# IceLab-X/FidelityFusion

Measured on AMD Instinct MI355X. Metric: GP NLML+Cholesky throughput (NxN fp64 GF/s, %MFMA-roofline) at N=16384, higher is better.
Workload: dtype f64; 1 GPU; headline: single-fidelity cigp NLML forward, ARD kernel, 1 block of N=16384 D=16 d=1 (BASELINE configs[2]); N=16384, D=16, d=1, blocks=1, blocks_in_flight_per_rank=1, parallelism=fidelity-shard x1 (LPT partition, one 8-byte all-reduce per step)

## Files before the change

fidelityfusion_amd/csrc/ffgp_internal.h:

```cpp
#pragma once
#include <hip/hip_runtime.h>
#include <cstdint>
#include <cstdio>
#include <cstdlib>
#include <cstring>
#include <vector>

#include "../../include/ffgp.h"

typedef double d4_t __attribute__((ext_vector_type(4)));
typedef double d2_t __attribute__((ext_vector_type(2)));

#define FFGP_NB 128
#define FFGP_MAX_STAGES 16

#define FFGP_HIP(call)                                                                        \
  do {                                                                                        \
    hipError_t e_ = (call);                                                                   \
    if (e_ != hipSuccess) {                                                                   \
      fprintf(stderr, "[ffgp] HIP error %s at %s:%d\n", hipGetErrorString(e_), __FILE__, __LINE__); \
      return FFGP_ERR_HIP;                                                                    \
    }                                                                                         \
  } while (0)

#define FFGP_CHECK(call)            \
  do {                              \
    int s_ = (call);                \
    if (s_ != 0) return s_;         \
  } while (0)

#define FFGP_GRAD_LANES 4
static inline int ffgp_round_up(int x, int m) { return (x + m - 1) / m * m; }

__device__ __forceinline__ double ffgp_kfun_val(int kind, double rinv, double s) {
  if (kind == FFGP_KFUN_SE) return exp(-0.5 * s);
  if (kind == FFGP_KFUN_MATERN12) return exp(-sqrt(s) * rinv);
  if (kind == FFGP_KFUN_MATERN32) {
    const double a = sqrt(3.0 * s) * rinv;
    return (1.0 + a) * exp(-a);
  }
  if (kind == FFGP_KFUN_RQ) return pow(1.0 + 0.5 * s * rinv, -1.0 / rinv);
  const double a = sqrt(5.0 * s) * rinv;
  return (1.0 + a + (5.0 / 3.0) * s * rinv * rinv) * exp(-a);
}
__device__ __forceinline__ double ffgp_kfun_m2d(int kind, double rinv, double s) {
  if (kind == FFGP_KFUN_SE) return exp(-0.5 * s);
  if (kind == FFGP_KFUN_MATERN12) {
    const double r = sqrt(s);
    return rinv / r * exp(-r * rinv);
  }
  if (kind == FFGP_KFUN_MATERN32) return 3.0 * rinv * rinv * exp(-sqrt(3.0 * s) * rinv);
  if (kind == FFGP_KFUN_RQ) return pow(1.0 + 0.5 * s * rinv, -1.0 / rinv - 1.0);
  const double a = sqrt(5.0 * s) * rinv;
  return (5.0 / 3.0) * rinv * rinv * (1.0 + a) * exp(-a);
}
__device__ __forceinline__ double ffgp_kfun_dparam(int kind, double rinv, double s, double phi) {
  if (kind != FFGP_KFUN_RQ) return 0.0;
  const double u = 0.5 * s * rinv;
  return phi * (u / (1.0 + u) - log1p(u));
}

__attribute__((weak)) __constant__ double ffgp_exp_coef[14] = {1.0, 1.0, 0.5, 1.0 / 6, 1.0 / 24, 1.0 / 120, 1.0 / 720, 1.0 / 5040, 1.0 / 40320, 1.0 / 362880,
                                         1.0 / 3628800, 1.0 / 39916800, 1.0 / 479001600, 1.0 / 6227020800.0};
struct ExpCoef {
  double c[14];
};
__device__ __forceinline__ void ffgp_exp_load(ExpCoef& e) {
#pragma unroll
  for (int i = 0; i < 14; ++i) e.c[i] = ffgp_exp_coef[i];
}
__device__ __forceinline__ double ffgp_exp_fast(double x, const ExpCoef& e) {
  x = fmax(x, -750.0);
  const double n = __builtin_rint(x * 1.4426950408889634);
  double r = __builtin_fma(n, -6.93147180369123816490e-01, x);
  r = __builtin_fma(n, -1.90821492927058770002e-10, r);
  double p = e.c[13];
#pragma unroll
  for (int i = 12; i >= 0; --i) p = __builtin_fma(p, r, e.c[i]);
  return __builtin_amdgcn_ldexp(p, (int)n);
}

__device__ __forceinline__ int ffgp_pow2_exp(double m) {
  if (!(m > 0.0)) return 0;
  const int e = ((__double2hiint(m) >> 20) & 0x7ff) - 1023;
  return min(max(e, -1021), 1021);
}

enum { OP_KMAJOR = 0, OP_MNMAJOR = 1 };
enum { TILES_FULL = 0, TILES_LOWER = 1 };

struct GemmArgs {
  const double* A;
  const double* B;
  double* C;
  int m, n, k;
  int lda, ldb, ldc;
  double alpha, beta;
// ... 295 lines not shown
```

fidelityfusion_amd/csrc/gemm.hip:

```cpp
#include <algorithm>

#include "ffgp_internal.h"
#include "diag_block.h"

#define BK 16
#ifndef FFGP_PD_SMALL
#define FFGP_PD_SMALL 4
#endif

#ifdef FFGP_GEMM_TRACE
__device__ unsigned long long* ffgp_trace_buf = nullptr;
extern "C" int ffgp_debug_set_trace(void* p) {
  return hipMemcpyToSymbol(HIP_SYMBOL(ffgp_trace_buf), &p, sizeof(p)) == hipSuccess ? 0 : -1;
}
#define FFGP_TRACE(slot)                                                                            \
  do {                                                                                              \
    if (tid == 0 && ffgp_trace_buf) {                                                               \
      ffgp_trace_buf[(size_t)bid * 8 + (slot)] = __builtin_readcyclecounter();                      \
      if ((slot) == 0) {                                                                            \
        unsigned hwid = 0, xcc = 0;                                                                 \
        asm volatile("s_getreg_b32 %0, hwreg(HW_REG_HW_ID)" : "=s"(hwid));                          \
        asm volatile("s_getreg_b32 %0, hwreg(HW_REG_XCC_ID)" : "=s"(xcc));                          \
        ffgp_trace_buf[(size_t)bid * 8 + 6] = ((unsigned long long)xcc << 32) | hwid;               \
        ffgp_trace_buf[(size_t)bid * 8 + 7] = wall_clock64();                                       \
// ... 185 lines not shown
  d4_t acc[WM][WN];
  if (load_c) {
#pragma unroll
    for (int i = 0; i < WM; ++i)
#pragma unroll
      for (int r = 0; r < 4; ++r) {
        const char* rowb = baseC + (size_t)(i * 4 + r) * row4_bytes;
#pragma unroll
        for (int j = 0; j < WN; ++j) acc[i][j][r] = *reinterpret_cast<const double*>(rowb + voffC + j * 128);
      }
  } else {
#pragma unroll
    for (int i = 0; i < WM; ++i)
#pragma unroll
      for (int j = 0; j < WN; ++j) acc[i][j] = (d4_t){0.0, 0.0, 0.0, 0.0};
  }
  sstore<OPA, TM>(smem, tid, ra[0]);
  sstore<OPB, TN>(smem + BUFA, tid, rb[0]);
  __syncthreads();
#ifdef FFGP_GEMM_TRACE
  if (tid == 0 && ffgp_trace_buf) ffgp_trace_buf[(size_t)trace_bid * 8 + 1] = __builtin_readcyclecounter();
#endif
  baseA += (size_t)PD * stepA;
  baseB += (size_t)PD * stepB;
  for (int kt0 = 0; kt0 < nkt; kt0 += PD) {
#pragma unroll
    for (int u = 0; u < PD; ++u) {
      const int kt = kt0 + u;
      if (kt >= nkt) break;
      const int par = (PD == 1) ? (kt & 1) : (u & 1);
      const double* sA = smem + par * STAGE;
      const double* sB = sA + BUFA;
      if (kt + PD < nkt) {
        gload_fast<TM>(baseA, voffA, ra[u]);
        gload_fast<TN>(baseB, voffB, rb[u]);
        baseA += stepA;
        baseB += stepB;
      }
#pragma unroll
      for (int kq = 0; kq < 4; ++kq) {
        double a[WM], b[WN];
#pragma unroll
        for (int i = 0; i < WM; ++i) a[i] = sA[offA[kq] + i * subA];
#pragma unroll
        for (int j = 0; j < WN; ++j) b[j] = sB[offB[kq] + j * subB];
#pragma unroll
        for (int i = 0; i < WM; ++i)
#pragma unroll
          for (int j = 0; j < WN; ++j)
            acc[i][j] = __builtin_amdgcn_mfma_f64_16x16x4f64(a[i], b[j], acc[i][j], 0, 0, NEG ? 1 : 0);
      }
      if (kt + 1 < nkt) {
        double* dA = smem + (par ^ 1) * STAGE;
        sstore<OPA, TM>(dA, tid, ra[(u + 1) % PD]);
        sstore<OPB, TN>(dA + BUFA, tid, rb[(u + 1) % PD]);
      }
      __syncthreads();
    }
  }
#ifdef FFGP_GEMM_TRACE
  if (tid == 0 && ffgp_trace_buf) ffgp_trace_buf[(size_t)trace_bid * 8 + 2] = __builtin_readcyclecounter();
#endif
#pragma unroll
  for (int i = 0; i < WM; ++i)
#pragma unroll
    for (int r = 0; r < 4; ++r) {
      char* rowb = baseC + (size_t)(i * 4 + r) * row4_bytes;
#pragma unroll
      for (int j = 0; j < WN; ++j) *reinterpret_cast<double*>(rowb + voffC + j * 128) = acc[i][j][r];
    }
}

typedef unsigned gemm_v4u __attribute__((ext_vector_type(4)));
__device__ __forceinline__ __amdgpu_buffer_rsrc_t gemm_rsrc(const char* base) {
  return __builtin_amdgcn_make_buffer_rsrc(const_cast<char*>(base), 0, 0xffffffff, 0x00020000);
}
template <int TS>
__device__ __forceinline__ void gload_buf(__amdgpu_buffer_rsrc_t r, const unsigned (&voff)[Geo<TS>::NLD], d2_t (&v)[Geo<TS>::NLD]) {
#pragma unroll
  for (int i = 0; i < Geo<TS>::NLD; ++i) v[i] = __builtin_bit_cast(d2_t, (gemm_v4u)__builtin_amdgcn_raw_buffer_load_b128(r, (int)voff[i], 0, 0));
}

typedef __attribute__((address_space(3))) char gemm_lds_t;
__device__ __forceinline__ void dma_lane_offsets(int tid, const unsigned (&voff)[4], unsigned (&dv)[4]) {
#pragma unroll
  for (int i = 0; i < 4; ++i) {
    const int idx = tid + 256 * i;
    const int row = idx >> 3, slot = idx & 7;
    dv[i] = voff[i] + (unsigned)(((slot ^ ((row >> 1) & 7)) - slot) * 16);
  }
}
__device__ __forceinline__ void gemm_dma16(__amdgpu_buffer_rsrc_t r, gemm_lds_t* dst, unsigned voff, int soff) {
  __builtin_amdgcn_raw_ptr_buffer_load_lds(r, dst, 16, (int)voff, soff, 0, 0);
}
#define DMA_BARRIER() asm volatile("s_waitcnt vmcnt(0) lgkmcnt(0)\n\ts_barrier" ::: "memory")

template <int OPA, int OPB, bool NEG, bool DIAG = false>
__device__ __forceinline__ void gemm_tile_fast128(const char* __restrict__ baseA, const char* __restrict__ baseB, size_t stepA, size_t stepB,
                                                  char* __restrict__ baseC, size_t row4_bytes, unsigned voffC, bool load_c, double* smem,
                                                  int nkt, int tid, const unsigned (&voffA)[4], const unsigned (&voffB)[4],
                                                  const int (&offA)[4], const int (&offB)[4], int trace_bid, double alpha = 0.0,
                                                  double beta = 0.0) {
  constexpr int TS = 128, W = 4;
  const int wave_d = DIAG ? __builtin_amdgcn_readfirstlane(tid >> 6) : 0;
  const bool mma = !DIAG || wave_d != 1;
  constexpr int BUFA = opbuf<OPA, TS>(), BUFB = opbuf<OPB, TS>(), STAGE = BUFA + BUFB;
  constexpr int subA = (OPA == OP_KMAJOR) ? 256 : 16;
  constexpr int subB = (OPB == OP_KMAJOR) ? 256 : 16;
#define GEMM_PIN() __builtin_amdgcn_sched_barrier(0)
#define GEMM_READ(st, kq, a, b)                                         \
  do {                                                                  \
    _Pragma("unroll") for (int i = 0; i < W; ++i) a[i] = (st)[offA[kq] + i * subA];        \
    _Pragma("unroll") for (int j = 0; j < W; ++j) b[j] = (st)[BUFA + offB[kq] + j * subB]; \
    GEMM_PIN();                                                         \
  } while (0)
#define GEMM_MFMA(a, b)                                                 \
  do {                                                                  \
    if (!DIAG || mma) {                                                 \
      _Pragma("unroll") for (int i = 0; i < W; ++i)                     \
        _Pragma("unroll") for (int j = 0; j < W; ++j)                   \
          acc[i][j] = __builtin_amdgcn_mfma_f64_16x16x4f64(a[i], b[j], acc[i][j], 0, 0, NEG ? 1 : 0);  \
    }                                                                   \
    GEMM_PIN();                                                         \
  } while (0)
  constexpr bool DMA = (OPA == OP_KMAJOR && OPB == OP_KMAJOR);
  [[maybe_unused]] const __amdgpu_buffer_rsrc_t rsA = gemm_rsrc(baseA), rsB = gemm_rsrc(baseB);
  [[maybe_unused]] unsigned dvA[4], dvB[4];
  [[maybe_unused]] gemm_lds_t* ldsw = nullptr;
  if constexpr (DMA) {
    dma_lane_offsets(tid, voffA, dvA);
    dma_lane_offsets(tid, voffB, dvB);
    ldsw = (gemm_lds_t*)smem + __builtin_amdgcn_readfirstlane(tid >> 6) * 1024;
  }
#define GEMM_DMA(p, stage, kt)                                          \
  gemm_dma16((p) < 4 ? rsA : rsB, ldsw + (stage) * (STAGE * 8) + ((p) < 4 ? 0 : BUFA * 8) + ((p) & 3) * 4096, \
             (p) < 4 ? dvA[(p) & 3] : dvB[(p) & 3], (kt) * (BK * 8))
#define GEMM_DMA_ALL(stage, kt)                                         \
  do {                                                                  \
    _Pragma("unroll") for (int p_ = 0; p_ < 8; ++p_) GEMM_DMA(p_, stage, kt); \
    GEMM_PIN();                                                         \
  } while (0)
#define GEMM_MFMA_DMA(a, b, stage, kt)                                  \
  do {                                                                  \
    if constexpr (DIAG) {       \
      GEMM_DMA_ALL(stage, kt);                                          \
      GEMM_MFMA(a, b);                                                  \
    } else {                                                            \
      _Pragma("unroll") for (int i = 0; i < W; ++i)                     \
        _Pragma("unroll") for (int j = 0; j < W; ++j) {                 \
          acc[i][j] = __builtin_amdgcn_mfma_f64_16x16x4f64(a[i], b[j], acc[i][j], 0, 0, NEG ? 1 : 0); \
          if (i * W + j < 8) {                                          \
            GEMM_PIN();                                                 \
            GEMM_DMA(i * W + j, stage, kt);                             \
            GEMM_PIN();                                                 \
          }                                                             \
        }                                                               \
      GEMM_PIN();                                                       \
    }                                                                   \
  } while (0)
  [[maybe_unused]] d2_t ra[4], rb[4];
  if constexpr (DMA) {
    GEMM_DMA_ALL(0, 0);
    if (nkt > 1) GEMM_DMA_ALL(1, 1);
  } else {
    gload_buf<TS>(rsA, voffA, ra);
    gload_buf<TS>(rsB, voffB, rb);
  }
  d4_t acc[W][W];
  if (load_c) {
// ... 66 lines not shown
      GEMM_PIN();
      GEMM_READ(sS, 1, ya, yb);
      GEMM_MFMA(xa, xb);
      GEMM_READ(sS, 2, xa, xb);
      GEMM_MFMA(ya, yb);
      sstore<OPA, TS>(sN, tid, ra);
      sstore<OPB, TS>(sN + BUFA, tid, rb);
      GEMM_PIN();
      GEMM_READ(sS, 3, ya, yb);
      GEMM_MFMA(xa, xb);
      LDS_BARRIER();
      GEMM_PIN();
      GEMM_READ(sN, 0, xa, xb);
      GEMM_MFMA(ya, yb);
    }
  }
  {
    const double* sS = smem + ((nkt - 1) & 1) * STAGE;
    GEMM_READ(sS, 1, ya, yb);
    GEMM_MFMA(xa, xb);
    GEMM_READ(sS, 2, xa, xb);
    GEMM_MFMA(ya, yb);
    GEMM_READ(sS, 3, ya, yb);
    GEMM_MFMA(xa, xb);
    GEMM_MFMA(ya, yb);
  }
#undef GEMM_PIN
#undef GEMM_READ
#undef GEMM_MFMA
#undef GEMM_DMA
#undef GEMM_DMA_ALL
#undef GEMM_MFMA_DMA
#ifdef FFGP_GEMM_TRACE
  if (tid == 0 && ffgp_trace_buf) ffgp_trace_buf[(size_t)trace_bid * 8 + 2] = __builtin_readcyclecounter();
#endif
  if constexpr (DIAG) {
    if (!mma) return;
    const bool below = wave_d == 2;
    const int lrow = (tid & 63) >> 4, lcol = tid & 15;
    const bool use_c = (beta != 0.0);
    double cv[2][4][W];
    auto load_group = [&](int i, double (&dst)[4][W]) {
#pragma unroll
      for (int r = 0; r < 4; ++r) {
        const char* rowb = baseC + (size_t)(i * 4 + r) * row4_bytes;
#pragma unroll
        for (int j = 0; j < W; ++j) dst[r][j] = *reinterpret_cast<const double*>(rowb + voffC + j * 128);
      }
    };
    if (use_c) {
      load_group(0, cv[0]);
    } else {
#pragma unroll
      for (int b = 0; b < 2; ++b)
#pragma unroll
        for (int r = 0; r < 4; ++r)
#pragma unroll
          for (int j = 0; j < W; ++j) cv[b][r][j] = 0.0;
    }
#pragma unroll
    for (int i = 0; i < W; ++i) {
      if (use_c && i + 1 < W) load_group(i + 1, cv[(i + 1) & 1]);
#pragma unroll
      for (int r = 0; r < 4; ++r) {
        char* rowb = baseC + (size_t)(i * 4 + r) * row4_bytes;
#pragma unroll
        for (int j = 0; j < W; ++j)
          if (below || i > j || (i == j && 4 * r + lrow >= lcol))
            *reinterpret_cast<double*>(rowb + voffC + j * 128) = alpha * acc[i][j][r] + beta * cv[i & 1][r][j];
      }
    }
    return;
  }
#pragma unroll
  for (int i = 0; i < W; ++i)
#pragma unroll
    for (int r = 0; r < 4; ++r) {
      char* rowb = baseC + (size_t)(i * 4 + r) * row4_bytes;
#pragma unroll
      for (int j = 0; j < W; ++j) *reinterpret_cast<double*>(rowb + voffC + j * 128) = acc[i][j][r];
    }
}

template <int OPA, int OPB, int TM, int TN, bool GUARD>
__device__ __forceinline__ void gemm_mainloop(const GemmArgs& p, const double* __restrict__ Ag, const double* __restrict__ Bg,
                                              double* smem, int m0, int n0, int kt0, int kt1, int tid,
                                              const int (&offA)[4], const int (&offB)[4],
                                              d4_t (&acc)[Geo<TM>::WT][Geo<TN>::WT]) {
  constexpr int WM = Geo<TM>::WT, WN = Geo<TN>::WT;
  constexpr int BUFA = opbuf<OPA, TM>(), BUFB = opbuf<OPB, TN>(), STAGE = BUFA + BUFB;
  constexpr int subA = (OPA == OP_KMAJOR) ? 256 : 16;
  constexpr int subB = (OPB == OP_KMAJOR) ? 256 : 16;
  d2_t ra[Geo<TM>::NLD], rb[Geo<TN>::NLD];
  gload<OPA, TM, GUARD>(Ag, p.lda, m0, p.m, kt0 * BK, p.k, tid, p.avec != 0, ra);
  gload<OPB, TN, GUARD>(Bg, p.ldb, n0, p.n, kt0 * BK, p.k, tid, p.bvec != 0, rb);
  sstore<OPA, TM>(smem, tid, ra);
  sstore<OPB, TN>(smem + BUFA, tid, rb);
  __syncthreads();
  for (int kt = kt0; kt < kt1; ++kt) {
    const int par = (kt - kt0) & 1;
    const double* sA = smem + par * STAGE;
    const double* sB = sA + BUFA;
    const bool more = (kt + 1 < kt1);
    if (more) {
      gload<OPA, TM, GUARD>(Ag, p.lda, m0, p.m, (kt + 1) * BK, p.k, tid, p.avec != 0, ra);
      gload<OPB, TN, GUARD>(Bg, p.ldb, n0, p.n, (kt + 1) * BK, p.k, tid, p.bvec != 0, rb);
    }
#pragma unroll
    for (int kq = 0; kq < 4; ++kq) {
      double a[WM], b[WN];
#pragma unroll
      for (int i = 0; i < WM; ++i) a[i] = sA[offA[kq] + i * subA];
#pragma unroll
      for (int j = 0; j < WN; ++j) b[j] = sB[offB[kq] + j * subB];
#pragma unroll
      for (int i = 0; i < WM; ++i)
#pragma unroll
        for (int j = 0; j < WN; ++j) acc[i][j] = __builtin_amdgcn_mfma_f64_16x16x4f64(a[i], b[j], acc[i][j], 0, 0, 0);
    }
    if (more) {
      double* dA = smem + (par ^ 1) * STAGE;
      sstore<OPA, TM>(dA, tid, ra);
      sstore<OPB, TN>(dA + BUFA, tid, rb);
    }
    __syncthreads();
  }
}

template <int OPA, int OPB, int MODE, int TM, int TN>
__device__ __forceinline__ void gemm_one_tile(const GemmArgs& p, const double* __restrict__ Ag, const double* __restrict__ Bg,
                                              double* __restrict__ Cg, double* smem, int ti, int tj, const int tid, const int bid,
                                              const bool general = false) {
  constexpr int WM = Geo<TM>::WT, WN = Geo<TN>::WT;
  const int lane = tid & 63, wave = tid >> 6;
  const int wm = wave >> 1, wn = wave & 1;
  int offA[4], offB[4];
  frag_offsets<OPA, TM>(lane, wm * (TM / 2), offA);
  frag_offsets<OPB, TN>(lane, wn * (TN / 2), offB);
  const bool fast_ab = p.fast && p.avec && p.bvec;
  const int m0 = ti * TM, n0 = tj * TN;

  int kbeg = 0, kend = p.k;
  if (p.lo_i) kbeg = max(kbeg, ti * TM);
  if (p.lo_j) kbeg = max(kbeg, tj * TN);
  if (p.hi_i) kend = min(kend, (ti + 1) * TM);
  if (p.hi_j) kend = min(kend, (tj + 1) * TN);
  const int kt0 = kbeg / BK;
  const int kt1 = (kend + BK - 1) / BK;

  const bool interior = (m0 + TM <= p.m) && (n0 + TN <= p.n) && (kt1 * BK <= p.k) && p.avec && p.bvec;
  if constexpr (TM == 128 && TN == 128 && OPA == OP_KMAJOR && OPB == OP_KMAJOR) {
    if (p.pack && fast_ab && interior && kt0 == 0 && kt1 * BK == p.k && !(MODE == TILES_LOWER && m0 < n0 + TN)) return;
  }
  const bool diag = (MODE == TILES_LOWER && m0 < n0 + TN);
  constexpr bool DIAG_FAST = (TM == 128 && TN == 128 && MODE == TILES_LOWER && OPA == OP_KMAJOR && OPB == OP_KMAJOR);
  if (fast_ab && interior && kt0 < kt1 && !general && (!diag || (DIAG_FAST && p.light))) {
    const size_t k0 = (size_t)kt0 * BK;
    const char* bA = reinterpret_cast<const char*>(Ag) +
                     ((OPA == OP_KMAJOR) ? ((size_t)m0 * p.lda + k0) : (k0 * p.lda + m0)) * 8;
    const char* bB = reinterpret_cast<const char*>(Bg) +
                     ((OPB == OP_KMAJOR) ? ((size_t)n0 * p.ldb + k0) : (k0 * p.ldb + n0)) * 8;
    const size_t stepA = (OPA == OP_KMAJOR) ? (size_t)BK * 8 : (size_t)BK * p.lda * 8;
    const size_t stepB = (OPB == OP_KMAJOR) ? (size_t)BK * 8 : (size_t)BK * p.ldb * 8;
    char* bC = reinterpret_cast<char*>(Cg) + ((size_t)m0 * p.ldc + n0) * 8;
    const size_t row4 = (size_t)p.ldc * 32;
    constexpr int PD = (TM == 128) ? 1 : FFGP_PD_SMALL;
    unsigned voffA[Geo<TM>::NLD], voffB[Geo<TN>::NLD];
    lane_byte_offsets<OPA, TM>(p.lda, tid, voffA);
    lane_byte_offsets<OPB, TN>(p.ldb, tid, voffB);
    const unsigned voffC = (unsigned)((wm * (TM / 2) + (lane >> 4)) * p.ldc + wn * (TN / 2) + (lane & 15)) * 8u;
    if constexpr (TM == 128 && TN == 128) {
      if constexpr (DIAG_FAST) {
        if (diag) {
          gemm_tile_fast128<OPA, OPB, false, true>(bA, bB, stepA, stepB, bC, row4, voffC, false, smem, kt1 - kt0, tid, voffA, voffB, offA, offB, bid,
                                                   p.alpha, p.beta);
          FFGP_TRACE(3);
          return;
        }
      }
      if (p.alpha < 0.0)
        gemm_tile_fast128<OPA, OPB, true>(bA, bB, stepA, stepB, bC, row4, voffC, p.beta != 0.0, smem, kt1 - kt0, tid, voffA, voffB, offA, offB, bid);
      else
        gemm_tile_fast128<OPA, OPB, false>(bA, bB, stepA, stepB, bC, row4, voffC, p.beta != 0.0, smem, kt1 - kt0, tid, voffA, voffB, offA, offB, bid);
    } else if (p.alpha < 0.0)
      gemm_tile_fast<OPA, OPB, TM, TN, true, PD>(bA, bB, stepA, stepB, bC, row4, voffC, p.beta != 0.0, smem, kt1 - kt0, tid, voffA,
                                             voffB, offA, offB, bid);
    else
      gemm_tile_fast<OPA, OPB, TM, TN, false, PD>(bA, bB, stepA, stepB, bC, row4, voffC, p.beta != 0.0, smem, kt1 - kt0, tid, voffA,
                                              voffB, offA, offB, bid);
    FFGP_TRACE(3);
    return;
  }

  d4_t acc[WM][WN];
#pragma unroll
  for (int i = 0; i < WM; ++i)
#pragma unroll
    for (int j = 0; j < WN; ++j) acc[i][j] = (d4_t){0.0, 0.0, 0.0, 0.0};

  if (kt0 < kt1) {
    if (interior)
      gemm_mainloop<OPA, OPB, TM, TN, false>(p, Ag, Bg, smem, m0, n0, kt0, kt1, tid, offA, offB, acc);
    else
      gemm_mainloop<OPA, OPB, TM, TN, true>(p, Ag, Bg, smem, m0, n0, kt0, kt1, tid, offA, offB, acc);
  }

  FFGP_TRACE(2);
  const double alpha = p.alpha, beta = p.beta;
  const bool use_c = (beta != 0.0);
  const int rbase0 = m0 + wm * (TM / 2) + (lane >> 4);
  const int cbase = n0 + wn * (TN / 2) + (lane & 15);
  double cv[2][4][WN];
  auto load_group = [&](int i, double (&dst)[4][WN]) {
#pragma unroll
    for (int r = 0; r < 4; ++r) {
      const int rowc = min(rbase0 + i * 16 + 4 * r, p.m - 1);
#pragma unroll
      for (int j = 0; j < WN; ++j) {
        const int colc = min(cbase + j * 16, p.n - 1);
        dst[r][j] = Cg[(size_t)rowc * p.ldc + colc];
      }
    }
  };
  if (use_c) {
    load_group(0, cv[0]);
  } else {
#pragma unroll
    for (int b = 0; b < 2; ++b)
#pragma unroll
      for (int r = 0; r < 4; ++r)
#pragma unroll
        for (int j = 0; j < WN; ++j) cv[b][r][j] = 0.0;
  }
#pragma unroll
  for (int i = 0; i < WM; ++i) {
    if (use_c && i + 1 < WM) load_group(i + 1, cv[(i + 1) & 1]);
#pragma unroll
    for (int r = 0; r < 4; ++r) {
      const int row = rbase0 + i * 16 + 4 * r;
#pragma unroll
      for (int j = 0; j < WN; ++j) {
        const int col = cbase + j * 16;
        if (row < p.m && col < p.n && (MODE != TILES_LOWER || col <= row)) {
          Cg[(size_t)row * p.ldc + col] = alpha * acc[i][j][r] + beta * cv[i & 1][r][j];
        }
      }
    }
  }
  FFGP_TRACE(3);
}

template <int PD>
__device__ __forceinline__ void gemm_slab16(const GemmArgs& p, const double* __restrict__ Ag, const double* __restrict__ Bg,
                                            double* __restrict__ Cg, double* smem, int m0, int n0, const int tid, const int bid) {
  constexpr int BUFA = 16 * 16, BUFB = opbuf<OP_KMAJOR, 128>(), STAGE = BUFA + BUFB;
  static_assert((PD & 1) == 0, "even prefetch depth: the LDS stage parity is compile-time");
  const int lane = tid & 63;
  const int wave = __builtin_amdgcn_readfirstlane(tid >> 6);
  int offA[4], offB[4];
  frag_offsets<OP_KMAJOR, 128>(lane, 0, offA);
  frag_offsets<OP_KMAJOR, 128>(lane, wave * 32, offB);
  const int nkt = p.k / BK;
  const bool has_a = wave < 2;
  const int arow = (tid >> 3) & 15, ach = tid & 7;
  const char* pA = reinterpret_cast<const char*>(Ag) + ((size_t)min(m0 + arow, p.m - 1) * p.lda + ach * 2) * 8;
  const int sa = arow * 16 + ((ach ^ ((arow >> 1) & 7)) << 1);
// ... 34 lines not shown
#pragma unroll
      for (int kq = 0; kq < 4; ++kq) {
        const double a = sA[offA[kq]];
        const double b0 = sB[offB[kq]], b1 = sB[offB[kq] + 256];
        acc[0] = __builtin_amdgcn_mfma_f64_16x16x4f64(a, b0, acc[0], 0, 0, 0);
        acc[1] = __builtin_amdgcn_mfma_f64_16x16x4f64(a, b1, acc[1], 0, 0, 0);
      }
      if (kt + 1 < nkt) {
        double* dA = smem + ((u & 1) ^ 1) * STAGE;
        if (has_a) *reinterpret_cast<d2_t*>(dA + sa) = ra[(u + 1) % PD];
        sstore<OP_KMAJOR, 128>(dA + BUFA, tid, rb[(u + 1) % PD]);
      }
      __syncthreads();
    }
  }
  FFGP_TRACE(2);
  const double alpha = p.alpha, beta = p.beta;
  const bool use_c = (beta != 0.0);
  const int row0 = m0 + (lane >> 4);
  const int col0 = n0 + wave * 32 + (lane & 15);
  double cv[4][2];
#pragma unroll
  for (int r = 0; r < 4; ++r) {
    const int rowc = min(row0 + 4 * r, p.m - 1);
#pragma unroll
    for (int j = 0; j < 2; ++j) cv[r][j] = use_c ? Cg[(size_t)rowc * p.ldc + col0 + j * 16] : 0.0;
  }
#pragma unroll
  for (int r = 0; r < 4; ++r) {
    const int row = row0 + 4 * r;
    if (row < p.m) {
#pragma unroll
      for (int j = 0; j < 2; ++j) Cg[(size_t)row * p.ldc + col0 + j * 16] = alpha * acc[j][r] + beta * cv[r][j];
    }
  }
  FFGP_TRACE(3);
}

template <int OPA, int OPB, int MODE, int TM, int TN>
__device__ __forceinline__ void gemm_block(const GemmArgs& p, const double* __restrict__ Ag, const double* __restrict__ Bg,
                                           double* __restrict__ Cg, double* smem, const int tid, const int bid) {
  FFGP_TRACE(0);
  if constexpr (TM == 128 && TN == 128 && MODE == TILES_LOWER && OPA == OP_KMAJOR && OPB == OP_KMAJOR) {
    if (bid >= p.slab_at) {
      const int s = bid - p.slab_at;
      const int mw = p.tiles_m * 128;
      const int per = (p.m - mw + 15) >> 4;
      const int tj = __builtin_amdgcn_readfirstlane(s / per);
      const int sl = __builtin_amdgcn_readfirstlane(s - tj * per);
      FFGP_TRACE_TILE(p.tiles_m, tj, 16);
      gemm_slab16<FFGP_PD_SMALL>(p, Ag, Bg, Cg, smem, mw + 16 * sl, tj * 128, tid, bid);
      return;
    }
  }
  if constexpr (TM == 128 && TN == 128) {
    if (bid >= p.split_at) {
      const int q = bid - p.split_at;
      int Ti, Tj;
      decode_tile(p.split_at + (q >> 2), MODE, p.tiles_m, p.tiles_n, Ti, Tj, p.band_log2);
      const int ti = __builtin_amdgcn_readfirstlane(2 * Ti + ((q >> 1) & 1));
      const int tj = __builtin_amdgcn_readfirstlane(2 * Tj + (q & 1));
      if (ti * 64 >= p.m || tj * 64 >= p.n || (MODE == TILES_LOWER && tj > ti)) return;
      FFGP_TRACE_TILE(ti, tj, 64);
      gemm_one_tile<OPA, OPB, MODE, 64, 64>(p, Ag, Bg, Cg, smem, ti, tj, tid, bid, MODE == TILES_LOWER && Ti == Tj);
      return;
    }
  }
  int t = bid;
  if (!(p.lo_i | p.lo_j | p.hi_i | p.hi_j)) {
    const int nwg = p.total_tiles;
    const int q = nwg >> 3, r = nwg & 7, xcd = bid & 7;
    t = (xcd < r ? xcd * (q + 1) : r * (q + 1) + (xcd - r) * q) + (bid >> 3);
  }
  int ti, tj;
  decode_tile(t, MODE, p.tiles_m, p.tiles_n, ti, tj, p.band_log2);
  ti = __builtin_amdgcn_readfirstlane(ti);
  tj = __builtin_amdgcn_readfirstlane(tj);
  FFGP_TRACE_TILE(ti, tj, TM);
  gemm_one_tile<OPA, OPB, MODE, TM, TN>(p, Ag, Bg, Cg, smem, ti, tj, tid, bid);
}

template <int OPA, int OPB, int MODE, int TAG, int TM, int TN>
__global__ __launch_bounds__(256, 2) void ffgp_gemm_f64(GemmArgs p) {
  __shared__ __attribute__((aligned(16))) double smem[2 * (opbuf<OPA, TM>() + opbuf<OPB, TN>())];
  const int tid = threadIdx.x;
  if (p.pub_word && tid == 0 && blockIdx.x == 0 && blockIdx.y == 0 && blockIdx.z == 0)
    __hip_atomic_store(p.pub_word, p.pub_val, __ATOMIC_RELAXED, __HIP_MEMORY_SCOPE_SYSTEM);
  if (p.prio) __builtin_amdgcn_s_setprio(2);
  const double* __restrict__ Ag = p.A + (size_t)blockIdx.y * p.sA + (size_t)blockIdx.z * p.sA2;
  const double* __restrict__ Bg = p.B + (size_t)blockIdx.y * p.sB + (size_t)blockIdx.z * p.sB2;
  double* __restrict__ Cg = p.C + (size_t)blockIdx.y * p.sC + (size_t)blockIdx.z * p.sC2;
  gemm_block<OPA, OPB, MODE, TM, TN>(p, Ag, Bg, Cg, smem, tid, blockIdx.x);
}

template <int OPA, int OPB, int MODE, int TAG, int TM, int TN>
__global__ __launch_bounds__(256, 2) void ffgp_gemm_f64_rag(GemmRag q) {
  __shared__ __attribute__((aligned(16))) double smem[2 * (opbuf<OPA, TM>() + opbuf<OPB, TN>())];
  const int tid = threadIdx.x;
  const GemmRagMember& r = q.mem[blockIdx.y];
  if ((int)blockIdx.x >= r.grid) return;
  if (q.base.prio) __builtin_amdgcn_s_setprio(2);
  GemmArgs p = q.base;
  p.A = r.A; p.B = r.B; p.C = r.C;
  p.m = r.m; p.n = r.n; p.k = r.k;
  p.lda = r.lda; p.ldb = r.ldb; p.ldc = r.ldc;
  p.tiles_m = r.tiles_m; p.tiles_n = r.tiles_n; p.total_tiles = r.total_tiles;
  p.grid = r.grid; p.split_at = r.split_at; p.slab_at = r.slab_at; p.light = r.light;
  p.fast = r.fast; p.avec = r.avec; p.bvec = r.bvec;
  gemm_block<OPA, OPB, MODE, TM, TN>(p, p.A, p.B, p.C, smem, tid, blockIdx.x);
}

#define GEMM_BAND_LOG2 3
#define POLITE_PAD_KB 40
template <int OPA, int OPB, int MODE, int TAG, int TM, int TN>
static int launch_t(ffgp_handle* h, const GemmArgs& a) {
  if (a.pad_lds > 0)
    FFGP_HIP(hipFuncSetAttribute(reinterpret_cast<const void*>(&ffgp_gemm_f64<OPA, OPB, MODE, TAG, TM, TN>),
                                 hipFuncAttributeMaxDynamicSharedMemorySize, 64 * 1024));
  hipLaunchKernelGGL((ffgp_gemm_f64<OPA, OPB, MODE, TAG, TM, TN>), dim3(a.grid, a.batch, a.batch2), dim3(256), a.pad_lds, h->stream, a);
  return FFGP_OK;
}

template <int TS>
static int dispatch(ffgp_handle* h, int opa, int opb, int mode, int syrk_tag, const GemmArgs& a) {
  if (syrk_tag) {
    if (opa == OP_KMAJOR && opb == OP_KMAJOR && mode == TILES_LOWER) return launch_t<OP_KMAJOR, OP_KMAJOR, TILES_LOWER, 1, TS, TS>(h, a);
  } else if (mode == TILES_LOWER) {
    if (opa == OP_KMAJOR && opb == OP_KMAJOR) return launch_t<OP_KMAJOR, OP_KMAJOR, TILES_LOWER, 0, TS, TS>(h, a);
    if (opa == OP_MNMAJOR && opb == OP_MNMAJOR) return launch_t<OP_MNMAJOR, OP_MNMAJOR, TILES_LOWER, 0, TS, TS>(h, a);
  } else {
    if (opa == OP_KMAJOR && opb == OP_KMAJOR) return launch_t<OP_KMAJOR, OP_KMAJOR, TILES_FULL, 0, TS, TS>(h, a);
    if (opa == OP_KMAJOR && opb == OP_MNMAJOR) return launch_t<OP_KMAJOR, OP_MNMAJOR, TILES_FULL, 0, TS, TS>(h, a);
    if (opa == OP_MNMAJOR && opb == OP_MNMAJOR) return launch_t<OP_MNMAJOR, OP_MNMAJOR, TILES_FULL, 0, TS, TS>(h, a);
    if (opa == OP_MNMAJOR && opb == OP_KMAJOR) return launch_t<OP_MNMAJOR, OP_KMAJOR, TILES_FULL, 0, TS, TS>(h, a);
  }
  return FFGP_ERR_ARG;
}

static inline bool aligned16(const void* p) { return (reinterpret_cast<uintptr_t>(p) & 15) == 0; }

static int count_tiles(int mode, int m, int n, int tsm, int tsn, int& tm, int& tn) {
  tm = (m + tsm - 1) / tsm;
  tn = (n + tsn - 1) / tsn;
  if (mode != TILES_LOWER) return tm * tn;
  int total = 0;
  for (int ti = 0; ti < tm; ++ti) total += (ti + 1 < tn) ? ti + 1 : tn;
  return total;
}

__global__ __launch_bounds__(256) void ffgp_splitk_reduce(const double* __restrict__ P, int ldp, long sP, int parts, double* __restrict__ C,
                                                         int ldc, int m, int n, double beta) {
  const long e = (long)blockIdx.x * 256 + threadIdx.x;
  if (e >= (long)m * n) return;
  const int r = (int)(e / n), c = (int)(e - (long)r * n);
  double acc = 0.0;
  const double* p = P + (size_t)r * ldp + c;
  for (int s = 0; s < parts; ++s) acc += p[(size_t)s * sP];
  double* dst = C + (size_t)r * ldc + c;
  *dst = (beta != 0.0) ? acc + beta * *dst : acc;
}

static int ensure_skw(ffgp_handle* h, size_t bytes) {
  if (bytes <= h->skw_bytes) return FFGP_OK;
  if (h->skw) {
    hipStreamSynchronize(h->stream);
    if (h->aux) hipStreamSynchronize(h->aux);
    hipFree(h->skw);
  }
  h->skw = nullptr;
  h->skw_bytes = 0;
  const size_t gran = (size_t)16 << 20;
  const size_t want = (bytes + gran - 1) / gran * gran;
  if (hipMalloc(&h->skw, want) != hipSuccess) return FFGP_ERR_ALLOC;
  h->skw_bytes = want;
  ++h->alloc_epoch;
  return FFGP_OK;
}

struct SkinnyArgs {
  const double* A;
// ... 498 lines not shown
```

fidelityfusion_amd/csrc/handle.hip:

```cpp
#include <atomic>
#include <iterator>
#include <cmath>
#include <strings.h>

#include "drivers.h"

#define SCAL_DOUBLES 2048

static const char* k_stage_names[FFGP_MAX_STAGES] = {"assemble", "potrf", "reduce", "trtri", "lauum", "grad",
                                                     "predict_gemm", "", "", "", "", "", "", "", "", ""};

int ffgp_ensure_ws(ffgp_handle* h, size_t bytes) {
  if (bytes <= h->ws_bytes) return FFGP_OK;
  if (h->ws) {
    hipStreamSynchronize(h->stream);
    hipFree(h->ws);
    h->ws = nullptr;
    h->ws_bytes = 0;
  }
  const size_t gran = (size_t)64 << 20;
  const size_t want = (bytes + gran - 1) / gran * gran;
  if (hipMalloc(&h->ws, want) != hipSuccess) {
    fprintf(stderr, "[ffgp] workspace allocation of %zu bytes failed\n", want);
    (void)hipGetLastError();
// ... 95 lines not shown
  for (int i = 0; i <= FFGP_MAX_STAGES; ++i) FFGP_HIP(hipEventCreate(&h->ev[i]));
  FFGP_HIP(hipEventCreate(&h->syrk_ev[0]));
  FFGP_HIP(hipEventCreate(&h->syrk_ev[1]));
  return FFGP_OK;
}

int ffgp_ensure_aux2(ffgp_handle* h) {
  if (h->aux2) return FFGP_OK;
  FFGP_HIP(hipStreamCreateWithFlags(&h->aux2, hipStreamNonBlocking));
  FFGP_HIP(hipStreamCreateWithFlags(&h->aux3, hipStreamNonBlocking));
  for (int i = 0; i < 2; ++i) FFGP_HIP(hipEventCreateWithFlags(&h->tri_ev[i], hipEventDisableTiming));
  return FFGP_OK;
}

extern "C" int ffgp_prepare_streams(ffgp_handle* h) {
  if (!h) return FFGP_ERR_ARG;
  FFGP_HIP(hipSetDevice(h->device));
  FFGP_CHECK(ffgp_ensure_aux2(h));
  FFGP_HIP(hipMemsetAsync(h->d_info + 8, 0, sizeof(int), h->aux));
  FFGP_HIP(hipMemsetAsync(h->d_info + 9, 0, sizeof(int), h->aux2));
  FFGP_HIP(hipMemsetAsync(h->d_info + 10, 0, sizeof(int), h->aux3));
  FFGP_HIP(hipStreamSynchronize(h->aux));
  FFGP_HIP(hipStreamSynchronize(h->aux2));
  FFGP_HIP(hipStreamSynchronize(h->aux3));
  return FFGP_OK;
}

static std::atomic<int> g_live_handles{0};
extern "C++" int ffgp_live_handles() { return g_live_handles.load(std::memory_order_relaxed); }

static bool env_on(const char* key) {
  const char* v = getenv(key);
  return v && *v && strcmp(v, "0") && strcasecmp(v, "false") && strcasecmp(v, "off");
}
static int default_ho_values() {
  const char* f = getenv("FFGP_HANDOFF");
  if (f && !strcmp(f, "events")) return 0;
  if (f && !strcmp(f, "values")) return 1;
  static const char* const serialising[] = {"ROCPROF_COUNTER_COLLECTION", "ROCPROF_COUNTERS", "ROCPROF_COUNTER_GROUPS", "ROCPROF_ADVANCED_THREAD_TRACE",
                                            "ROCP_METRICS", "ROCPROFILER_METRICS_PATH", "HIP_LAUNCH_BLOCKING", "CUDA_LAUNCH_BLOCKING",
                                            "AMD_SERIALIZE_KERNEL", "AMD_SERIALIZE_COPY"};
  for (const char* k : serialising)
    if (env_on(k)) return 0;
  const char* tools = getenv("HSA_TOOLS_LIB");
  if (tools && (strstr(tools, "rocprofiler64") || strstr(tools, "libroctracer"))) return 0;
  return 1;
}

int ffgp_create(int device, ffgp_handle** out) {
  if (!out) return FFGP_ERR_ARG;
  int count = 0;
  if (hipGetDeviceCount(&count) != hipSuccess || count <= 0 || device < 0 || device >= count) {
    fprintf(stderr, "[ffgp] no usable HIP device (requested %d of %d); libffgp has no CPU fallback\n", device, count);
    return FFGP_ERR_NODEVICE;
  }
  FFGP_HIP(hipSetDevice(device));
  ffgp_handle* h = new ffgp_handle();
  h->device = device;
  h->lookahead = 1;
  h->small_tile_threshold = 640;
  h->batch_grad_ob = 1;
  h->tile32_threshold = 1024;
  h->polite_m = 8192;
  h->split_rem_max = 180;
  h->syrk_light_tiles = 1;
  h->super_block = 1024;
  h->splitk_min_k = 1024;
  h->tlin_gemm_min = 8192;
  h->skinny_max_n = 8;
  h->super_min_n = 2048;
  h->la_carry = 2;
  h->la_carry_n = 12288;
  h->la_carry_rows = 8192;
  h->la_min_n = 1024;
  h->chase_xl = 1;
  h->chase_xl_max_n = 2048;
  {
    static std::atomic<int> next_xcc{0};
    h->chase_xcc = next_xcc.fetch_add(1) & 7;
  }
  h->aux_prio = 1;
  h->nb_outer = 512;
  h->trsm128 = 1;
  h->polite64_pad_kb = 60;
  h->polite32_pad_kb = 46;
  h->ho_values = default_ho_values();
  h->ho_defer = 2;
  h->ho_gate = 1;
  h->grad_lanes = 3;
  h->ho_timeout_ms = 2000;
  h->ho_defer_slot = -1;
  h->ho_gdefer_slot = -1;
  h->diag_excl_rows = 4096;
  h->trsm128_max_m = 8192;
  h->trtri_overlap = 1;
  h->small2_off = 1;
  h->q2_split_min_cols = 8192;
  h->sb_lower = 1;
  h->sb_lower_min_n = 6144;
  h->sb_sym_wg = 2048;
  h->asm_mm = 1;
  h->asm_mm_min = 6144;
  h->asm_mm_grid = 768;
  const int rc = create_resources(h);
  if (rc != FFGP_OK) {
    ffgp_destroy(h);
    return rc;
  }
  g_live_handles.fetch_add(1, std::memory_order_relaxed);
  h->counted_live = 1;
  *out = h;
  return FFGP_OK;
}

int ffgp_destroy(ffgp_handle* h) {
  if (!h) return FFGP_OK;
  if (h->counted_live) {
    g_live_handles.fetch_sub(1, std::memory_order_relaxed);
    h->counted_live = 0;
  }
  hipSetDevice(h->device);
  if (h->own) hipStreamSynchronize(h->own);
  if (h->aux) hipStreamSynchronize(h->aux);
  if (h->ws) hipFree(h->ws);
  if (h->dinv) hipFree(h->dinv);
  if (h->sinv) hipFree(h->sinv);
  if (h->tsw) hipFree(h->tsw);
  if (h->skw) hipFree(h->skw);
  if (h->ews) hipFree(h->ews);
  if (h->d_link) hipFree(h->d_link);
  if (h->aux2) hipStreamDestroy(h->aux2);
  if (h->aux3) hipStreamDestroy(h->aux3);
  if (h->ev_switch) hipEventDestroy(h->ev_switch);
  for (int i = 0; i < 2; ++i)
    if (h->tri_ev[i]) hipEventDestroy(h->tri_ev[i]);
  if (h->d_info) hipFree(h->d_info);
  if (h->ho_mem) hipFree(h->ho_mem);
  if (h->bt_info) hipFree(h->bt_info);
  if (h->train_g) hipFree(h->train_g);
  if (h->train_tree) hipFree(h->train_tree);
  for (int z = 0; z < FFGP_GRAD_LANES; ++z) {
    if (h->lane_ev[z]) hipEventDestroy(h->lane_ev[z]);
    if (z > 0 && h->lane_skw[z]) hipFree(h->lane_skw[z]);
  }
  if (h->lane_scal) hipFree(h->lane_scal);
  if (h->small_kbuf) hipFree(h->small_kbuf);
  if (h->train_blk) hipFree(h->train_blk);
  if (h->train_blk_host) hipHostFree(h->train_blk_host);
  ffgp_assemble_collect_free(h);
  if (h->bt_info_host) hipHostFree(h->bt_info_host);
  if (h->d_scal) hipFree(h->d_scal);
  if (h->d_asm) hipFree(h->d_asm);
  ffgp_rawg_drop(h->fwdg);
  if (h->fwdg) {
    if (h->fwdg->stage) hipFree(h->fwdg->stage);
    delete h->fwdg;
    h->fwdg = nullptr;
  }
  if (h->h_info) hipHostFree(h->h_info);
  if (h->h_scal) hipHostFree(h->h_scal);
  for (int i = 0; i <= FFGP_MAX_STAGES; ++i)
    if (h->ev[i]) hipEventDestroy(h->ev[i]);
  for (int i = 0; i < 2; ++i)
    if (h->syrk_ev[i]) hipEventDestroy(h->syrk_ev[i]);
  for (hipEvent_t e : h->syrk_pool) hipEventDestroy(e);
  for (int i = 0; i < 10; ++i)
    if (h->la_ev[i]) hipEventDestroy(h->la_ev[i]);
  if (h->aux) hipStreamDestroy(h->aux);
// ... 139 lines not shown
```

Measured before the change: 55920 GF/s.

## Add multi-stage LDS DMA ring pipeline for 64 and 32 GEMM tiles

Adds a ring-buffered GEMM tile path for 64x64 and 32x32 k-major tiles. It uses buffer-load-to-LDS DMA with a configurable stage count, partial vmcnt waits and explicitly interleaved MFMA and DMA issue. LDS sizing now scales with the stage count, and the polite-kernel LDS padding is derived from it, so total occupancy stays unchanged. With the default ring depth of 2 this mainly replaces the register-staged path with direct DMA. That risks different scheduling behaviour on the small tiles.

```diff
diff --git a/fidelityfusion_amd/csrc/ffgp_internal.h b/fidelityfusion_amd/csrc/ffgp_internal.h
--- a/fidelityfusion_amd/csrc/ffgp_internal.h
+++ b/fidelityfusion_amd/csrc/ffgp_internal.h
@@ -13,6 +13,14 @@
 
 #define FFGP_NB 128
 #define FFGP_MAX_STAGES 16
+#ifndef FFGP_RING64
+#define FFGP_RING64 2
+#endif
+#ifndef FFGP_RING32
+#define FFGP_RING32 2
+#endif
+#define FFGP_POLITE64_LDS_KB 92
+#define FFGP_POLITE32_LDS_KB 62
 
 #define FFGP_HIP(call)                                                                        \
   do {                                                                                        \
diff --git a/fidelityfusion_amd/csrc/gemm.hip b/fidelityfusion_amd/csrc/gemm.hip
--- a/fidelityfusion_amd/csrc/gemm.hip
+++ b/fidelityfusion_amd/csrc/gemm.hip
@@ -291,9 +291,10 @@
 }
 
 typedef __attribute__((address_space(3))) char gemm_lds_t;
-__device__ __forceinline__ void dma_lane_offsets(int tid, const unsigned (&voff)[4], unsigned (&dv)[4]) {
-#pragma unroll
-  for (int i = 0; i < 4; ++i) {
+template <int N>
+__device__ __forceinline__ void dma_lane_offsets(int tid, const unsigned (&voff)[N], unsigned (&dv)[N]) {
+#pragma unroll
+  for (int i = 0; i < N; ++i) {
     const int idx = tid + 256 * i;
     const int row = idx >> 3, slot = idx & 7;
     dv[i] = voff[i] + (unsigned)(((slot ^ ((row >> 1) & 7)) - slot) * 16);
@@ -526,6 +527,211 @@
     }
 }
 
+template <int OPA, int OPB, int TM, int TN>
+constexpr int gemm_stages() {
+  return (OPA == OP_KMAJOR && OPB == OP_KMAJOR && TM == TN && TM == 64) ? FFGP_RING64
+         : (OPA == OP_KMAJOR && OPB == OP_KMAJOR && TM == TN && TM == 32) ? FFGP_RING32 : 2;
+}
+template <int VM>
+__device__ __forceinline__ void dma_barrier_keep() {
+  asm volatile("s_waitcnt vmcnt(%0) lgkmcnt(0)\n\ts_barrier" ::"n"(VM) : "memory");
+}
+
+template <int TS, bool NEG, int S>
+__device__ __forceinline__ void gemm_tile_ring(const char* __restrict__ baseA, const char* __restrict__ baseB, char* __restrict__ baseC,
+                                               size_t row4_bytes, unsigned voffC, bool load_c, double* smem, int nkt, int tid,
+                                               const unsigned (&voffA)[Geo<TS>::NLD], const unsigned (&voffB)[Geo<TS>::NLD],
+                                               const int (&offA)[4], const int (&offB)[4], int trace_bid) {
+  constexpr int W = Geo<TS>::WT, NP = Geo<TS>::NLD, P = 2 * NP;
+  constexpr int BUF = TS * 16, STAGE = 2 * BUF;
+  static_assert((TS == 64 || TS == 32) && S >= 2 && S <= 8 && (S - 2) * P < 64, "ring depth");
+  static_assert(TS != 64 || S * STAGE * 8 <= 65536, "the 128-tile kernels' split tail runs the 64-tile ring in their 64 KiB");
+  const __amdgpu_buffer_rsrc_t rsA = gemm_rsrc(baseA), rsB = gemm_rsrc(baseB);
+  unsigned dvA[NP], dvB[NP];
+  dma_lane_offsets(tid, voffA, dvA);
+  dma_lane_offsets(tid, voffB, dvB);
+  gemm_lds_t* const ldsw = (gemm_lds_t*)smem + __builtin_amdgcn_readfirstlane(tid >> 6) * 1024;
+#define RING_PIN() __builtin_amdgcn_sched_barrier(0)
+#define RING_PIECE(p, st, kt)                                           \
+  gemm_dma16((p) < NP ? rsA : rsB, ldsw + (st) * (STAGE * 8) + ((p) < NP ? 0 : BUF * 8) + ((p) % NP) * 4096, \
+             (p) < NP ? dvA[(p) % NP] : dvB[(p) % NP], (kt) * (BK * 8))
+#pragma unroll
+  for (int s = 0; s < S; ++s)
+    if (s < nkt) {
+#pragma unroll
+      for (int p = 0; p < P; ++p) RING_PIECE(p, s, s);
+    }
+  RING_PIN();
+  d4_t acc[W][W];
+  if (load_c) {
+#pragma unroll
+    for (int i = 0; i < W; ++i)
+#pragma unroll
+      for (int r = 0; r < 4; ++r) {
+        const char* rowb = baseC + (size_t)(i * 4 + r) * row4_bytes;
+#pragma unroll
+        for (int j = 0; j < W; ++j) acc[i][j][r] = *reinterpret_cast<const double*>(rowb + voffC + j * 128);
+      }
+  } else {
+#pragma unroll
+    for (int i = 0; i < W; ++i)
+#pragma unroll
+      for (int j = 0; j < W; ++j) acc[i][j] = (d4_t){0.0, 0.0, 0.0, 0.0};
+  }
+  RING_PIN();
+  DMA_BARRIER();
+#pragma unroll
+  for (int i = 0; i < W; ++i)
+#pragma unroll
+    for (int j = 0; j < W; ++j) asm volatile("" : "+v"(acc[i][j]));
+#ifdef FFGP_GEMM_TRACE
+  if (tid == 0 && ffgp_trace_buf) ffgp_trace_buf[(size_t)trace_bid * 8 + 1] = __builtin_readcyclecounter();
+#endif
+  RING_PIN();
+  int st = 0;
+  if constexpr (TS == 64) {
+    double xa[W], xb[W], ya[W], yb[W];
+#define RING_READ(sp, kq, a, b)                                         \
+  do {                                                                  \
+    _Pragma("unroll") for (int i = 0; i < W; ++i) a[i] = (sp)[offA[kq] + i * 256];       \
+    _Pragma("unroll") for (int j = 0; j < W; ++j) b[j] = (sp)[BUF + offB[kq] + j * 256]; \
+    RING_PIN();                                                         \
+  } while (0)
+#define RING_MFMA(a, b)                                                 \
+  do {                                                                  \
+    _Pragma("unroll") for (int i = 0; i < W; ++i)                       \
+      _Pragma("unroll") for (int j = 0; j < W; ++j)                     \
+        acc[i][j] = __builtin_amdgcn_mfma_f64_16x16x4f64(a[i], b[j], acc[i][j], 0, 0, NEG ? 1 : 0);  \
+    RING_PIN();                                                         \
+  } while (0)
+#define RING_MFMA_PIECES(a, b, st_, kt_)                                \
+  do {                                                                  \
+    _Pragma("unroll") for (int i = 0; i < W; ++i)                       \
+      _Pragma("unroll") for (int j = 0; j < W; ++j) {                   \
+        acc[i][j] = __builtin_amdgcn_mfma_f64_16x16x4f64(a[i], b[j], acc[i][j], 0, 0, NEG ? 1 : 0); \
+        RING_PIN();                                                     \
+        RING_PIECE(i * W + j, st_, kt_);                                \
+        RING_PIN();                                                     \
+      }                                                                 \
+  } while (0)
+#define RING_KQ012(sS)                                                  \
+  do {                                                                  \
+    RING_READ(sS, 1, ya, yb);                                           \
+    RING_MFMA(xa, xb);                                                  \
+    RING_READ(sS, 2, xa, xb);                                           \
+    RING_MFMA(ya, yb);                                                  \
+    RING_READ(sS, 3, ya, yb);                                           \
+    RING_MFMA(xa, xb);                                                  \
+  } while (0)
+    RING_READ(smem, 0, xa, xb);
+    for (int kt = 0; kt + S < nkt; ++kt) {
+      const int sn = (st + 1 == S) ? 0 : st + 1;
+      const double* sS = smem + st * STAGE;
+      const double* sN = smem + sn * STAGE;
+      RING_KQ012(sS);
+      dma_barrier_keep<(S - 2) * P>();
+      RING_PIN();
+      RING_READ(sN, 0, xa, xb);
+      RING_MFMA_PIECES(ya, yb, st, kt + S);
+      st = sn;
+    }
+#define RING_TAIL(J)                                                    \
+  if constexpr ((J) < S) {                                              \
+    if ((J) >= S - nkt) {                                               \
+      const int sn = (st + 1 == S) ? 0 : st + 1;                        \
+      const double* sS = smem + st * STAGE;                             \
+      RING_KQ012(sS);                                                   \
+      if constexpr ((J) < S - 1) {                                      \
+        dma_barrier_keep<((S - 2 - (J)) > 0 ? (S - 2 - (J)) : 0) * P>(); \
+        RING_PIN();                                                     \
+        RING_READ(smem + sn * STAGE, 0, xa, xb);                        \
+      }                                                                 \
+      RING_MFMA(ya, yb);                                                \
+      st = sn;                                                          \
+    }                                                                   \
+  }
+    RING_TAIL(0) RING_TAIL(1) RING_TAIL(2) RING_TAIL(3) RING_TAIL(4) RING_TAIL(5) RING_TAIL(6) RING_TAIL(7)
+#undef RING_TAIL
+#undef RING_KQ012
+#undef RING_MFMA_PIECES
+#undef RING_MFMA
+#undef RING_READ
+  } else {
+    double ra[4], rb[4];
+#define RING_READ1(sp, kq)                                              \
+  do {                                                                  \
+    ra[kq] = (sp)[offA[kq]];                                            \
+    rb[kq] = (sp)[BUF + offB[kq]];                                      \
+    RING_PIN();                                                         \
+  } while (0)
+#define RING_MFMA1(kq)                                                  \
+  do {                                                                  \
+    acc[0][0] = __builtin_amdgcn_mfma_f64_16x16x4f64(ra[kq], rb[kq], acc[0][0], 0, 0, NEG ? 1 : 0);  \
+    RING_PIN();                                                         \
+  } while (0)
+    RING_READ1(smem, 0);
+    RING_READ1(smem, 1);
+    RING_READ1(smem, 2);
+    RING_READ1(smem, 3);
+    for (int kt = 0; kt + S < nkt; ++kt) {
+      const int sn = (st + 1 == S) ? 0 : st + 1;
+      const double* sN = smem + sn * STAGE;
+      RING_MFMA1(0);
+      RING_MFMA1(1);
+      dma_barrier_keep<(S - 2) * P>();
+      RING_PIN();
+      RING_READ1(sN, 0);
+      RING_READ1(sN, 1);
+      RING_MFMA1(2);
+      RING_PIECE(0, st, kt + S);
+      RING_PIN();
+      RING_READ1(sN, 2);
+      RING_MFMA1(3);
+      RING_PIECE(1, st, kt + S);
+      RING_PIN();
+      RING_READ1(sN, 3);
+      st = sn;
+    }
+#define RING_TAIL(J)                                                    \
+  if constexpr ((J) < S) {                                              \
+    if ((J) >= S - nkt) {                                               \
+      const int sn = (st + 1 == S) ? 0 : st + 1;                        \
+      [[maybe_unused]] const double* sN = smem + sn * STAGE;            \
+      RING_MFMA1(0);                                                    \
+      RING_MFMA1(1);                                                    \
+      if constexpr ((J) < S - 1) {                                      \
+        dma_barrier_keep<((S - 2 - (J)) > 0 ? (S - 2 - (J)) : 0) * P>(); \
+        RING_PIN();                                                     \
+        RING_READ1(sN, 0);                                              \
+        RING_READ1(sN, 1);                                              \
+      }                                                                 \
+      RING_MFMA1(2);                                                    \
+      if constexpr ((J) < S - 1) RING_READ1(sN, 2);                     \
+      RING_MFMA1(3);                                                    \
+      if constexpr ((J) < S - 1) RING_READ1(sN, 3);                     \
+      st = sn;                                                          \
+    }                                                                   \
+  }
+    RING_TAIL(0) RING_TAIL(1) RING_TAIL(2) RING_TAIL(3) RING_TAIL(4) RING_TAIL(5) RING_TAIL(6) RING_TAIL(7)
+#undef RING_TAIL
+#undef RING_MFMA1
+#undef RING_READ1
+  }
+#undef RING_PIECE
+#undef RING_PIN
+#ifdef FFGP_GEMM_TRACE
+  if (tid == 0 && ffgp_trace_buf) ffgp_trace_buf[(size_t)trace_bid * 8 + 2] = __builtin_readcyclecounter();
+#endif
+#pragma unroll
+  for (int i = 0; i < W; ++i)
+#pragma unroll
+    for (int r = 0; r < 4; ++r) {
+      char* rowb = baseC + (size_t)(i * 4 + r) * row4_bytes;
+#pragma unroll
+      for (int j = 0; j < W; ++j) *reinterpret_cast<double*>(rowb + voffC + j * 128) = acc[i][j][r];
+    }
+}
+
 template <int OPA, int OPB, int TM, int TN, bool GUARD>
 __device__ __forceinline__ void gemm_mainloop(const GemmArgs& p, const double* __restrict__ Ag, const double* __restrict__ Bg,
                                               double* smem, int m0, int n0, int kt0, int kt1, int tid,
@@ -608,7 +814,7 @@
     const size_t stepB = (OPB == OP_KMAJOR) ? (size_t)BK * 8 : (size_t)BK * p.ldb * 8;
     char* bC = reinterpret_cast<char*>(Cg) + ((size_t)m0 * p.ldc + n0) * 8;
     const size_t row4 = (size_t)p.ldc * 32;
-    constexpr int PD = (TM == 128) ? 1 : FFGP_PD_SMALL;
+    [[maybe_unused]] constexpr int PD = (TM == 128) ? 1 : FFGP_PD_SMALL;
     unsigned voffA[Geo<TM>::NLD], voffB[Geo<TN>::NLD];
     lane_byte_offsets<OPA, TM>(p.lda, tid, voffA);
     lane_byte_offsets<OPB, TN>(p.ldb, tid, voffB);
@@ -626,6 +832,12 @@
         gemm_tile_fast128<OPA, OPB, true>(bA, bB, stepA, stepB, bC, row4, voffC, p.beta != 0.0, smem, kt1 - kt0, tid, voffA, voffB, offA, offB, bid);
       else
         gemm_tile_fast128<OPA, OPB, false>(bA, bB, stepA, stepB, bC, row4, voffC, p.beta != 0.0, smem, kt1 - kt0, tid, voffA, voffB, offA, offB, bid);
+    } else if constexpr (TM == TN && (TM == 64 || TM == 32) && OPA == OP_KMAJOR && OPB == OP_KMAJOR) {
+      constexpr int S = gemm_stages<OPA, OPB, TM, TN>();
+      if (p.alpha < 0.0)
+        gemm_tile_ring<TM, true, S>(bA, bB, bC, row4, voffC, p.beta != 0.0, smem, kt1 - kt0, tid, voffA, voffB, offA, offB, bid);
+      else
+        gemm_tile_ring<TM, false, S>(bA, bB, bC, row4, voffC, p.beta != 0.0, smem, kt1 - kt0, tid, voffA, voffB, offA, offB, bid);
     } else if (p.alpha < 0.0)
       gemm_tile_fast<OPA, OPB, TM, TN, true, PD>(bA, bB, stepA, stepB, bC, row4, voffC, p.beta != 0.0, smem, kt1 - kt0, tid, voffA,
                                              voffB, offA, offB, bid);
@@ -826,7 +1038,7 @@
 
 template <int OPA, int OPB, int MODE, int TAG, int TM, int TN>
 __global__ __launch_bounds__(256, 2) void ffgp_gemm_f64(GemmArgs p) {
-  __shared__ __attribute__((aligned(16))) double smem[2 * (opbuf<OPA, TM>() + opbuf<OPB, TN>())];
+  __shared__ __attribute__((aligned(16))) double smem[gemm_stages<OPA, OPB, TM, TN>() * (opbuf<OPA, TM>() + opbuf<OPB, TN>())];
   const int tid = threadIdx.x;
   if (p.pub_word && tid == 0 && blockIdx.x == 0 && blockIdx.y == 0 && blockIdx.z == 0)
     __hip_atomic_store(p.pub_word, p.pub_val, __ATOMIC_RELAXED, __HIP_MEMORY_SCOPE_SYSTEM);
@@ -839,7 +1051,7 @@
 
 template <int OPA, int OPB, int MODE, int TAG, int TM, int TN>
 __global__ __launch_bounds__(256, 2) void ffgp_gemm_f64_rag(GemmRag q) {
-  __shared__ __attribute__((aligned(16))) double smem[2 * (opbuf<OPA, TM>() + opbuf<OPB, TN>())];
+  __shared__ __attribute__((aligned(16))) double smem[gemm_stages<OPA, OPB, TM, TN>() * (opbuf<OPA, TM>() + opbuf<OPB, TN>())];
   const int tid = threadIdx.x;
   const GemmRagMember& r = q.mem[blockIdx.y];
   if ((int)blockIdx.x >= r.grid) return;
diff --git a/fidelityfusion_amd/csrc/handle.hip b/fidelityfusion_amd/csrc/handle.hip
--- a/fidelityfusion_amd/csrc/handle.hip
+++ b/fidelityfusion_amd/csrc/handle.hip
@@ -201,8 +201,8 @@
   h->aux_prio = 1;
   h->nb_outer = 512;
   h->trsm128 = 1;
-  h->polite64_pad_kb = 60;
-  h->polite32_pad_kb = 46;
+  h->polite64_pad_kb = FFGP_POLITE64_LDS_KB - 16 * FFGP_RING64;
+  h->polite32_pad_kb = FFGP_POLITE32_LDS_KB - 8 * FFGP_RING32;
   h->ho_values = default_ho_values();
   h->ho_defer = 2;
   h->ho_gate = 1;
```

Result: no change. 56390 GF/s, median of 6 (+0.8%).
